# pytorch/audio

Hardware: AMD Instinct MI355X
Metric: audio-sec/sec MelSpectrogram (b=256, 16kHz, n_fft=400, n_mels=80) (higher is better)
Workload: dtype f32; 1 GPU; MelSpectrogram n_fft=400 hop=160 n_mels=80, batch=256 x 10 s @16 kHz fp32 per GPU (BASELINE configs[1]); per_gpu_batch=256

## Files before the change

### audio_amd/csrc/melspec400.h

```cpp
#pragma once
#include <cstdint>
#include <cstring>
#include <type_traits>
#include "hd.h"
#include "stft_generic.h"

namespace aamd {
namespace m400 {

constexpr int kN = 400;
constexpr int kPad = 200;
constexpr int kFramesPerWave = 6;
constexpr int kWavesPerBlock = 12;
constexpr int kMinWavesPerSimd = 3;
constexpr int kTOff[20] = {0, 260, 520, 652, 784, 916, 1444, 1576, 128, 388,
                           2104, 2232, 2364, 1708, 1840, 1048, 1180, 1312, 1972, 2492};
constexpr int kTBufDwords = 2492 + 128;
constexpr int kTRow = 44;
constexpr int kTPair = 20 * kTRow;
constexpr int kLdsDwordsPerWave = 3 * kTPair;
constexpr int kPK = 208;
constexpr int kPPair = 416;
constexpr int kSOff = 1344;

template <int H>
struct Hop {
  static constexpr int hop = 20 * H;
  static constexpr int nx = 20 + H;
  static constexpr int tile_samples = (kFramesPerWave - 1) * hop + kN;
  static constexpr int pair_stride = 2 * hop;
  static constexpr int pad = ((20 - pair_stride % 32) + 32) % 32;
  static constexpr int blk_data = pair_stride / 4, blk_pieces = blk_data + pad / 4;
  static constexpr int data_pieces = tile_samples / 4;
  static constexpr int pieces = data_pieces + (pad / 4) * ((tile_samples - 1) / pair_stride);
  static constexpr int ndma = (pieces + 63) / 64;
  static constexpr int lds_dwords = (kSOff + 256 * ndma > kLdsDwordsPerWave) ? kSOff + 256 * ndma : kLdsDwordsPerWave;
  static_assert(pad % 4 == 0 && (pair_stride + pad) % 32 == 20, "staging pad");
};
struct PcmStereo { uint32_t lr; };
template <typename TIn> struct InTraits {
  static constexpr int chans = 1;
  AAMD_HD static float get(const TIn* p, int) { return (float)*p; }
};
template <> struct InTraits<PcmStereo> {
  static constexpr int chans = 2;
  AAMD_HD static float get(const PcmStereo* p, int ch) { return (float)(int16_t)(uint16_t)(p->lr >> (16 * ch)); }
};

template <int H, typename TIn>
struct Stage {
  using HC = Hop<H>;
  static constexpr int spp = 16 / (int)sizeof(TIn);
  static constexpr int pair_dwords = HC::pair_stride * (int)sizeof(TIn) / 4;
  static constexpr int pad = sizeof(TIn) == 4 ? HC::pad : ((44 - pair_dwords % 64) + 64) % 64;
  static constexpr int pad_elems = pad * 4 / (int)sizeof(TIn);
  static constexpr int blk_data = HC::pair_stride / spp, blk_pieces = blk_data + pad / 4;
  static constexpr int data_pieces = HC::tile_samples / spp;
  static constexpr int pieces = data_pieces + (pad / 4) * ((HC::tile_samples - 1) / HC::pair_stride);
  static constexpr int ndma = (pieces + 63) / 64;
  static constexpr bool ok = (HC::pair_stride % spp == 0) && (HC::tile_samples % spp == 0) && (pad % 4 == 0) &&
                             (kSOff + 256 * ndma <= HC::lds_dwords);
};
static_assert(Stage<8, float>::blk_data == Hop<8>::blk_data && Stage<8, float>::blk_pieces == Hop<8>::blk_pieces &&
              Stage<8, float>::pieces == Hop<8>::pieces && Stage<8, float>::ndma == Hop<8>::ndma, "float staging = Hop");
static_assert(Stage<8, int16_t>::ok && Stage<8, int16_t>::pad == 12 && Stage<8, int16_t>::ndma == 3, "int16 staging, hop 160");
static_assert(Stage<10, int16_t>::ok && Stage<5, float>::ok && Stage<10, float>::ok, "staging geometry");
static_assert(sizeof(PcmStereo) == 4 && Stage<8, PcmStereo>::ok && Stage<10, PcmStereo>::ok &&
              Stage<8, PcmStereo>::pieces == Stage<8, float>::pieces, "interleaved stereo stages like float");

constexpr int kMelSlots = 20;
constexpr int kMelMaxRounds = 8;
constexpr int kMelMaxTaps = 64;

static_assert(3 * kPPair <= kLdsDwordsPerWave && 2 * kPK <= kPPair, "P rows must fit in the transposition buffer");
static_assert(kTBufDwords <= kLdsDwordsPerWave, "transposition rows must fit in the wave's region");
static_assert(3 * (kPK - 201) <= 64, "one lane per tail bin");
static_assert(Hop<8>::lds_dwords == kLdsDwordsPerWave && Hop<8>::ndma == 5 && Hop<8>::pad == 20, "headline geometry");

enum { EPI400_MEL = 0, EPI400_MEL_DB = 1, EPI400_SPEC = 2, EPI400_MEL_NORM = 3, EPI400_MFCC = 4 };
struct Epi400 {
  float multiplier, amin, db_sub;
  float* group_max;
  int64_t rows_per_group;
  float power;
  float gain;
  const float* mean;
  const float* invstd;
  int64_t out_frames;
  const float* dct_frag;
  int n_mfcc;
  float top_db;
  float* tile_min;
  int* fix_count;
  int* fix_list;
  int frag_in_lds;
  int fixup;
  int lab;
  unsigned* pool;
  int pool_p;
};
constexpr int kSpecBins = 201;

#ifndef AAMD_M400_POOLS
#define AAMD_M400_POOLS 0
#endif
constexpr int kPoolStride = 64;
constexpr unsigned kNoTile = 0xffffffffu;
AAMD_HD int pool_count(int nb) { return nb >= 8 ? nb / 8 : 1; }
AAMD_HD int pool_members(int nb, int np, int p) { return p < nb ? (nb - p + np - 1) / np : 0; }
AAMD_HD int pool_share(int tiles_per_block) { const int p = tiles_per_block / 20; return tiles_per_block < 48 ? 0 : p > 8 ? 8 : p; }
AAMD_HD unsigned pool_tile(int np, int P, int tiles_per_block, unsigned n_tiles, int p, int members, unsigned ticket,
                           bool& exhausted) {
  exhausted = ticket >= (unsigned)(members * P);
  if (exhausted) return kNoTile;
  const unsigned m = ticket / (unsigned)P, off = ticket - m * (unsigned)P;
  const unsigned long long t = (unsigned long long)(m * (unsigned)np + (unsigned)p) * (unsigned)tiles_per_block +
                               (unsigned)(tiles_per_block - P) + off;
  return t < n_tiles ? (unsigned)t : kNoTile;
}
static_assert(kFramesPerWave * kSpecBins + 3 <= kSOff && 3 * 2 * kSpecBins + 3 <= kSOff, "SPEC rows must fit below the staging area");

AAMD_HD constexpr int col_of_pos(int pi) {
  return pi == 0 ? 0 : pi == 1 ? 10 : (pi & 1) ? 20 - (pi >> 1) : (pi >> 1);
}
AAMD_HD constexpr int pos_of_col(int c) {
  return c == 0 ? 0 : c == 10 ? 1 : c < 10 ? 2 * c : 2 * (20 - c) + 1;
}

constexpr int kMfccMT = 3, kMfccMels = 80, kMfccSteps = 3;
constexpr float kMfccYScale = 1.0f / 16.0f, kMfccDScale = 16.0f;
static_assert(kMfccYScale * kMfccDScale == 1.0f, "the accumulators leave the matrix pipe unscaled");
constexpr int kMfccFragFloats = kMfccMT * kMfccSteps * 2 * 64 * 4;
AAMD_HD int mfcc_frag_piece(int t, int s, int hl, int lane) { return ((t * kMfccSteps + s) * 2 + hl) * 64 + lane; }
AAMD_HD int mfcc_slot_mel(int s, int lane, int j) {
  if (s < 2) return 32 * s + 8 * (lane >> 4) + j;
  return j < 4 ? 64 + 4 * (lane >> 4) + j : -1;
}
AAMD_HD float mfcc_frag_value(const float* dct, int n_mels, int n_mfcc, int t, int s, int lane, int j) {
  const int mel = mfcc_slot_mel(s, lane, j), coef = 16 * t + (lane & 15);
  return (mel >= 0 && mel < n_mels && coef < n_mfcc) ? dct[mel * n_mfcc + coef] * kMfccDScale : 0.0f;
}
AAMD_HD int mfcc_b_col_frame(int lane) { const int j = lane & 7; return j < kFramesPerWave ? j : kFramesPerWave - 1; }
AAMD_HD int mfcc_b_col_plane(int lane) { return (lane >> 3) & 1; }
AAMD_HD int mfcc_b_index(int lane, int s) {
  return mfcc_b_col_plane(lane) * (kFramesPerWave * kMfccMels) + mfcc_b_col_frame(lane) * kMfccMels +
         (s < 2 ? 32 * s + 8 * (lane >> 4) : 64 + 4 * (lane >> 4));
}
constexpr int kMfccPlaneHalves = kFramesPerWave * kMfccMels;

struct MelTab {
  const float* w;
  const int* lo2;
  const int* rc;
  const int* row_mel;
  int n_mels, ws, n_rounds;
};

AAMD_HD int mel_rounds(int n_mels) { return (n_mels + kMelSlots - 1) / kMelSlots; }
AAMD_HD int mel_ws(int max_width) {
  const int w4 = (max_width + 1 + 3) & ~3;
  return ((w4 >> 2) & 1) ? w4 : w4 + 4;
}
AAMD_HD int mel_rows(int n_mels) { return mel_rounds(n_mels) * kMelSlots; }
AAMD_HD int mel_tab_dwords(int n_mels, int max_width) {
  return mel_rows(n_mels) * (mel_ws(max_width) + 2) + kMelMaxRounds;
}
AAMD_HD int row_to_mel(const MelBandsDev& mb, int row) {
  const int m = mb.order ? mb.order[row] : row;
  return (m >= 0 && m < mb.n_mels) ? m : -1;
}

AAMD_HD void mel_tab_layout(const MelBandsDev& mb, float* base, MelTab& mt) {
  mt.n_mels = mb.n_mels;
  mt.ws = mel_ws(mb.max_width);
  mt.n_rounds = mel_rounds(mb.n_mels);
  const int rows = mel_rows(mb.n_mels);
  mt.w = base;
  int* lo2 = reinterpret_cast<int*>(base + rows * mt.ws);
  mt.lo2 = lo2;
  mt.row_mel = lo2 + rows;
  mt.rc = lo2 + 2 * rows;
}

AAMD_HD void mel_tab_rounds(int tid, int nthr, const MelBandsDev& mb, float* base, MelTab& mt) {
  mt.n_mels = mb.n_mels;
  mt.ws = mel_ws(mb.max_width);
  mt.n_rounds = mel_rounds(mb.n_mels);
  const int rows = mel_rows(mb.n_mels);
  mt.w = base;
  int* lo2 = reinterpret_cast<int*>(base + rows * mt.ws);
  int* row_mel = lo2 + rows;
  int* rc = row_mel + rows;
  mt.lo2 = lo2;
  mt.row_mel = row_mel;
  mt.rc = rc;
  for (int r = tid; r < mt.n_rounds; r += nthr) {
    int rw = 4;
    for (int row = r * kMelSlots; row < (r + 1) * kMelSlots; ++row) {
      const int q = row_to_mel(mb, row);
      if (q < 0) continue;
      const int e = (mb.width[q] + (mb.lo[q] & 1) + 3) & ~3;
      rw = e > rw ? e : rw;
    }
    rc[r] = rw >> 2;
  }
}

AAMD_HD void mel_tab_fill(int tid, int nthr, const MelBandsDev& mb, float* base, const MelTab& mt) {
  float* w = base;
  const int rows = mel_rows(mb.n_mels);
  int* lo2 = reinterpret_cast<int*>(base + rows * mt.ws);
  int* row_mel = lo2 + rows;
  for (int i = tid; i < rows * mt.ws; i += nthr) {
    const int row = i / mt.ws, j = i - row * mt.ws;
    const int m = row_to_mel(mb, row);
    const int rw = 4 * mt.rc[row / kMelSlots];
    const int lo = m >= 0 ? mb.lo[m] : 0, wd = m >= 0 ? mb.width[m] : 0;
    int l2 = lo & ~1;
    if (l2 + rw > kPK) l2 = kPK - rw;
    const int off = lo - l2;
    w[i] = (j >= off && j - off < wd) ? mb.weights[m * mb.max_width + (j - off)] : 0.0f;
    if (j == 0) {
      lo2[row] = l2;
      row_mel[row] = m;
    }
  }
}

constexpr int kTwRow = 42;
constexpr int kConstDwords = 20 * kTwRow + 20 * 20;

AAMD_HD void const_tab_build(int tid, int nthr, const float* window, const float* tw400, float scale,
                             float* base) {
  for (int i = tid; i < 20 * 20; i += nthr) {
    const int b = i / 20, s = i - 20 * b;
    const int idx = (b * s) % kN;
    base[kTwRow * b + 2 * s] = tw400[2 * idx];
    base[kTwRow * b + 2 * s + 1] = tw400[2 * idx + 1];
    base[20 * kTwRow + i] = window[b + 20 * s] * (0.5f * scale);
  }
}

AAMD_HD size_t lds_bytes(int n_mels, int max_width, int wave_dwords = kLdsDwordsPerWave, bool mfcc = false) {
  return ((size_t)kWavesPerBlock * wave_dwords + kConstDwords + mel_tab_dwords(n_mels, max_width) + 4 +
          (mfcc ? kMfccFragFloats : 0)) * sizeof(float);
}

struct LaneConst {
  const float* tw;
  const float* win;
  int p, pi, col;
  int active;
  int troff;
};

AAMD_HD void lane_init(int lane, const float* const_tab, LaneConst& c) {
  c.active = lane < 60;
  const int l = c.active ? lane : lane - 20;
  c.p = l / 20;
  c.pi = l - 20 * c.p;
  c.col = col_of_pos(c.pi);
  c.tw = const_tab + kTwRow * c.pi;
  c.win = const_tab + 20 * kTwRow + 20 * c.pi;
  int toff = 0;
#pragma unroll
  for (int k = 0; k < 20; ++k) toff = (c.col == k) ? kTOff[k] : toff;
  c.troff = toff + 20 * c.p;
}

AAMD_HD void dft4(float ar, float ai, float br, float bi, float cr, float ci, float dr, float di,
                  float* o_r, float* o_i) {
// ... 818 lines not shown
    for (int i = threadIdx.x; i < kMfccFragFloats; i += blockDim.x) frag_lds[i] = epi.dct_frag[i];
  if (EPI != EPI400_SPEC && mb.table400 != nullptr) {
    float* dst = const_tab + kConstDwords;
    for (int i = threadIdx.x; i < tab_dwords; i += blockDim.x) dst[i] = mb.table400[i];
    mel_tab_layout(mb, dst, mt);
    __syncthreads();
  } else {
    if (EPI != EPI400_SPEC) mel_tab_rounds(threadIdx.x, blockDim.x, mb, const_tab + kConstDwords, mt);
    __syncthreads();
    if (EPI != EPI400_SPEC) mel_tab_fill(threadIdx.x, blockDim.x, mb, const_tab + kConstDwords, mt);
    __syncthreads();
  }

  long long lab_t1 = 0;
  if (LAB & 1024) lab_t1 = wall_clock64();
  LaneConst c;
  lane_init(lane, const_tab, c);
  constexpr bool kWinRegs = (EPI != EPI400_MFCC || H != 10) && (((LAB & 8192) != 0) || !(LAB & 262144));
  float winr[20], twr[40];
  if (kWinRegs) {
#pragma unroll
    for (int q = 0; q < 20; ++q) winr[q] = c.win[q];
  }
  constexpr int kTwReg = 3, kTwRegPin = 4, kTwRegDb = 1, kTwRegMfcc = 2;
  constexpr bool kPlain = H == 8 && std::is_same<TIn, float>::value && LAB == 0;
  constexpr int kTwRegBatches = (LAB & 16384) ? 4
                                : (SIG != 0 && EPI == EPI400_MEL) ? ((AR & AR_PIN) ? kTwRegPin : kTwReg)
                                : !kPlain ? 0
                                : EPI == EPI400_SPEC ? 2
                                : (EPI == EPI400_MEL && SIG == 0) ? (NR <= 4 ? 1 : 3)
                                : (EPI == EPI400_MFCC && NR <= 4) ? kTwRegMfcc
                                : (EPI == EPI400_MEL_DB && NR <= 4) ? kTwRegDb : 0;
  if (kTwRegBatches > 0) {
#pragma unroll
    for (int q = 0; q < 10 * kTwRegBatches; ++q) twr[q] = c.tw[q];
  }
  constexpr bool kHoist = NR <= 4;
  MelRegs<NR> mregs;
  const MelRegs<NR>* mh = nullptr;
  if (EPI != EPI400_SPEC && kHoist) {
    mel_regs_load<NR>(c, mt, mregs);
    mh = &mregs;
  }
  if (SIG != 0) {
    static_assert(SIG == 0 || NR == 4, "filterbank signatures are 4 rounds of 20 mels");
    const int sig_rt = mregs.nc[0] | (mregs.nc[1 % NR] << 4) | (mregs.nc[2 % NR] << 8) | (mregs.nc[3 % NR] << 12);
    if (mt.n_rounds != NR || mt.n_mels != kMelSlots * NR || sig_rt != SIG) __builtin_trap();
  }
  if (EPI == EPI400_MFCC && (mt.n_rounds != NR || mt.n_mels != kMelSlots * NR)) __builtin_trap();
  float nrm_mean[NR], nrm_inv[NR];
  if (EPI == EPI400_MEL_NORM) {
#pragma unroll
    for (int r = 0; r < NR; ++r) {
      const int m = r < mt.n_rounds ? mt.row_mel[r * kMelSlots + c.pi] : -1;
      nrm_mean[r] = m >= 0 ? epi.mean[m] : 0.0f;
      nrm_inv[r] = m >= 0 ? epi.invstd[m] : 0.0f;
    }
  }
  const unsigned long long self_mask = __ballot((c.col == 0) || (c.col == 10));
  using SG = Stage<H, TIn>;
  static_assert(SG::ok, "no staging layout for this hop / input type");
  int spiece[SG::ndma];
#pragma unroll
  for (int k = 0; k < SG::ndma; ++k) spiece[k] = SG::spp * stage_src_piece<H, TIn>(64 * k + lane);

  const int nb = gridDim.x;
  int lb = blockIdx.x;
  if ((nb & 7) == 0) lb = (blockIdx.x & 7) * (nb >> 3) + (blockIdx.x >> 3);
  unsigned blk_first = (unsigned)lb * (unsigned)tiles_per_block;
  unsigned blk_count = 0;
  if (blk_first < (unsigned)n_tiles) {
    blk_count = (unsigned)n_tiles - blk_first;
    if (blk_count > (unsigned)tiles_per_block) blk_count = (unsigned)tiles_per_block;
  }
  if (EPI == EPI400_MFCC && epi.fixup != 0) {
    blk_first = 0;
    blk_count = fix_cnt;
  }
  const unsigned queue_addr = (unsigned)(uintptr_t)queue;
  auto claim = [&]() {
    int v = 0;
    if (lane == 0)
      asm volatile("ds_add_rtn_u32 %0, %1, %2\n\ts_waitcnt lgkmcnt(0)" : "=v"(v) : "v"(queue_addr), "v"(1) : "memory");
    return (unsigned)__builtin_amdgcn_readfirstlane(v);
  };
#if AAMD_M400_POOLS
#define AAMD_M400_POOLED (AAMD_M400_POOLS && (LAB == 0) && epi.pool != nullptr && !(EPI == EPI400_MFCC && epi.fixup != 0))
  if (AAMD_M400_POOLED && blk_count > (unsigned)(tiles_per_block - epi.pool_p)) blk_count = (unsigned)(tiles_per_block - epi.pool_p);
  unsigned pool_ticket = 0;
  auto pool_request = [&]() {
    int lbo = (int)(blk_first / (unsigned)tiles_per_block);
    asm volatile("" : "+s"(lbo));
    unsigned* const ctr = epi.pool + (lbo % pool_count(nb)) * kPoolStride;
    if (lane == 0) pool_ticket = __hip_atomic_fetch_add(ctr, 1u, __ATOMIC_RELAXED, __HIP_MEMORY_SCOPE_AGENT);
  };
  auto pool_take = [&]() {
    int lbo = (int)(blk_first / (unsigned)tiles_per_block);
    asm volatile("" : "+s"(lbo));
    const int np = pool_count(nb), pid = lbo % np, mem = pool_members(nb, np, pid);
    for (;;) {
      const unsigned v = (unsigned)__builtin_amdgcn_readfirstlane((int)pool_ticket);
      if (v + 1u == (unsigned)(mem * (epi.pool_p + kWavesPerBlock)) && lane == 0)
        __hip_atomic_store(epi.pool + pid * kPoolStride, 0u, __ATOMIC_RELAXED, __HIP_MEMORY_SCOPE_AGENT);
      bool exhausted;
      const unsigned t = pool_tile(np, epi.pool_p, tiles_per_block, (unsigned)n_tiles, pid, mem, v, exhausted);
      if (t != kNoTile) return t - blk_first;
      if (exhausted) return 0x80000000u;
      pool_request();
    }
  };
  constexpr unsigned kBadIdx = 0x80000000u, kPendIdx = 0x80000001u;
#define AAMD_M400_IDX_OK(I) ((((I) ^ 0x80000000u)) > 1u)
#define AAMD_M400_LOCAL(I) ((I) < blk_count ? (I) : kBadIdx)
#else
#define AAMD_M400_IDX_OK(I) ((I) < blk_count)
#define AAMD_M400_LOCAL(I) (I)
#endif
  constexpr unsigned kLabChunk = 8;
  unsigned* gq = reinterpret_cast<unsigned*>(epi.group_max);
  int g_pending = 0;
  unsigned g_base = 0, g_pos = 0;
  auto g_request = [&]() {
    if (lane == 0) g_pending = (int)__hip_atomic_fetch_add(gq, 1u, __ATOMIC_RELAXED, __HIP_MEMORY_SCOPE_AGENT);
  };
  if (LAB & 131072) {
    blk_count = (unsigned)n_tiles;
    g_request();
    g_base = (unsigned)__builtin_amdgcn_readfirstlane(g_pending) * kLabChunk;
    g_request();
  }
  auto g_next = [&]() {
    if (++g_pos < kLabChunk) return g_base + g_pos;
    g_base = (unsigned)__builtin_amdgcn_readfirstlane(g_pending) * kLabChunk;
    g_pos = 0;
    g_request();
    return g_base;
  };

  static_assert(kFramesPerWave * kHop >= kPad, "tile 1 starts inside the clip");
  unsigned tin_hi = 0;
  if (in_aligned && length >= kN - kPad) {
    int64_t last = (length - (kN - kPad)) / kHop - (kFramesPerWave - 1);
    if (last > (int64_t)n_frames - kFramesPerWave) last = (int64_t)n_frames - kFramesPerWave;
    if (last >= kFramesPerWave) tin_hi = (unsigned)(last / kFramesPerWave);
  }
  const int64_t out_row_elems =
      EPI == EPI400_SPEC   ? (int64_t)n_frames * (epi.power > 0.0f ? kSpecBins : 2 * kSpecBins)
      : EPI == EPI400_MFCC ? (int64_t)n_frames * epi.n_mfcc
                           : (EPI == EPI400_MEL_NORM ? epi.out_frames : (int64_t)n_frames) * (int64_t)mb.n_mels;
  auto tile_fill = [&](TileInfo& ti, unsigned idx) {
    ti.t0 = (int)ti.tin * kFramesPerWave;
    ti.staged = AAMD_M400_IDX_OK(idx) && ti.tin - 1u < tin_hi;
  };
  auto tile_info = [&](unsigned idx) {
    TileInfo ti;
    unsigned t = ((LAB & 131072) ? 0u : blk_first) + idx;
    if (EPI == EPI400_MFCC && epi.fixup != 0)
      t = idx < blk_count ? (unsigned)__hip_atomic_load(epi.fix_list + fix_base + idx, __ATOMIC_RELAXED, __HIP_MEMORY_SCOPE_AGENT) : 0u;
    const unsigned row = t / (unsigned)tiles_per_row;
    ti.row = row;
    ti.tin = t - row * (unsigned)tiles_per_row;
    ti.in_off = (ti.row / InTraits<TIn>::chans) * row_stride;
    ti.out_off = ti.row * out_row_elems;
    tile_fill(ti, idx);
    return ti;
  };
  constexpr bool kCarry = !(LAB & (131072 | 16777216)) && !AAMD_M400_POOLS && EPI != EPI400_MFCC && InTraits<TIn>::chans == 1;
  constexpr unsigned kCarryMinTiles = 16;
  auto tile_next = [&](const TileInfo& from, unsigned from_idx, unsigned idx) {
    if (!kCarry || (unsigned)tiles_per_row < kCarryMinTiles) return tile_info(idx);
    TileInfo ti = from;
    if (!(AAMD_M400_IDX_OK(idx))) {
      ti.staged = false;
      return ti;
    }
    ti.tin = from.tin + (idx - from_idx);
    while (ti.tin >= (unsigned)tiles_per_row) {
      ti.tin -= (unsigned)tiles_per_row;
      ti.row += 1;
      ti.in_off += row_stride;
      ti.out_off += out_row_elems;
    }
    tile_fill(ti, idx);
    return ti;
  };
  auto stage_issue = [&](const TileInfo& ti) {
    const TIn* src = wav + ti.in_off + ((int64_t)ti.t0 * kHop - kPad);
    if (LAB & 32) src = wav + 6 * kHop;
#pragma unroll
    for (int k = 0; k < SG::ndma; ++k)
      if (!(LAB & 64) || k == 0)
        glds16s(src, (unsigned)spiece[k] * (unsigned)sizeof(TIn), s_addr + 1024 * k);
  };

  float wmax = -INFINITY;
  int64_t wgroup = -1, wrow = -1;
  constexpr bool kDb = (EPI == EPI400_MEL_DB) || (EPI == EPI400_MFCC);
  const bool fix = (EPI == EPI400_MFCC) && epi.fixup != 0;
  auto flush_max = [&]() {
    if (kDb && !fix && epi.group_max != nullptr && wgroup >= 0) {
      float m = wmax;
#pragma unroll
      for (int off = 32; off > 0; off >>= 1) m = fmaxf(m, __shfl_xor(m, off, 64));
      if (lane == 0) atomic_max_f32(epi.group_max + wgroup, m);
    }
    wmax = -INFINITY;
  };

  if (kIoWave && wave >= kWavesPerBlock - kNio) {
    constexpr unsigned D = 8;
    constexpr bool kFetchOnly = (LAB & 134217728) != 0;
    if (!(LAB & 33554432)) {
      const unsigned n_mine = (blk_count + (unsigned)kNio - 1u - (unsigned)(wave - (kWavesPerBlock - kNio))) / (unsigned)kNio;
      for (unsigned i = 0; i < n_mine + D; ++i) {
        const unsigned t = i * (unsigned)kNio + (unsigned)(wave - (kWavesPerBlock - kNio));
        if (i < n_mine) {
          const TileInfo ti = tile_info(AAMD_M400_LOCAL(t));
          const unsigned dst = (unsigned)(uintptr_t)(smem400 + (t % (unsigned)kWavesPerBlock) * HC::lds_dwords + kSOff);
          if (ti.staged) {
            const TIn* src = wav + ti.in_off + ((int64_t)ti.t0 * kHop - kPad);
#pragma unroll
            for (int k = 0; k < SG::ndma; ++k) glds16(src + spiece[k], dst + 1024 * k);
          }
        }
        if (i >= D) {
          if (kFetchOnly) {
            asm volatile("s_waitcnt vmcnt(40)" ::: "memory");
          } else {
            asm volatile("s_waitcnt vmcnt(56)" ::: "memory");
            const unsigned told = t - D * (unsigned)kNio;
            const TileInfo to = tile_info(AAMD_M400_LOCAL(told));
            const float* stg = smem400 + (told % (unsigned)kWavesPerBlock) * HC::lds_dwords;
            store_wide(lane, mt, stg, out + to.row * (int64_t)n_frames * (int64_t)mb.n_mels, to.t0, n_frames);
          }
        }
      }
    }
    blk_count = 0;
  }
  unsigned cur_idx = (LAB & 131072) ? g_base : (unsigned)wave;
#if AAMD_M400_POOLS
  if (cur_idx >= blk_count) cur_idx = kBadIdx;
  if (AAMD_M400_POOLED && cur_idx == kBadIdx) {
    pool_request();
    cur_idx = pool_take();
  }
#endif
  TileInfo cur = tile_info(cur_idx);
  if (LAB & 128) {
    const int k = (wave + 6 * lb) % 3;
    for (int i = 0; i < k; ++i) __builtin_amdgcn_s_sleep(112);
  }
  if (LAB & 2048) {
    const int k = 4 * (wave & 3) + (wave >> 2) % 3;
    for (int i = 0; i < (k % 12); ++i) __builtin_amdgcn_s_sleep(17);
  }
  if (LAB & 4096) {
    const int k = 4 * ((wave >> 2) % 3) + (wave & 3);
    for (int i = 0; i < k; ++i) __builtin_amdgcn_s_sleep(17);
  }
  float Xn[HC::nx];
  auto gload = [&](const TileInfo& ti) {
    const TIn* src = wav + ti.in_off + ((int64_t)ti.t0 * kHop - kPad) + (HC::pair_stride * c.p + c.pi);
#pragma unroll
    for (int q = 0; q < HC::nx; ++q) Xn[q] = InTraits<TIn>::get(src + 20 * q, (int)(ti.row % InTraits<TIn>::chans));
  };
  if (LAB & 32768) {
#pragma unroll
    for (int q = 0; q < HC::nx; ++q) Xn[q] = 0.0f;
    if (cur.staged) gload(cur);
  } else if (cur.staged && !(LAB & 8) && !fix) {
    stage_issue(cur);
  }

  long long ph_acc[6] = {0, 0, 0, 0, 0, 0}, ph_t = 0;
  int ph_tiles = 0;
#define AAMD_M400_STAMP(K)                                  \
  if (LAB & 8388608) {                                      \
    const long long now_ = (long long)clock64();            \
    ph_acc[K] += now_ - ph_t;                               \
    ph_t = now_;                                            \
  }
  using mfcc_f32x4 = __attribute__((ext_vector_type(4))) float;
  mfcc_f32x4 cf[kMfccMT];
  const int mfcc_elab = (LAB & 524288) ? epi.lab : 0;
  auto mfcc_finish = [&](int64_t row, int64_t t0) {
#pragma unroll
    for (int t = 0; t < kMfccMT; ++t)
#pragma unroll
      for (int i = 0; i < 4; ++i) {
        cf[t][i] += __int_as_float(__builtin_amdgcn_mov_dpp(__float_as_int(cf[t][i]), 0x128, 0xf, 0xf, true));
        asm volatile("" : "+v"(cf[t][i]));
      }
    const int64_t left64 = n_frames - t0;
    const int left = left64 < kFramesPerWave ? (int)left64 : kFramesPerWave;
    if (!(LAB & 2) && !(mfcc_elab & 8) && (lane & 15) < left) {
      float* otile = out + (row * (int64_t)n_frames + t0) * (int64_t)epi.n_mfcc;
      const unsigned ooff = (unsigned)(lane & 15) * (unsigned)epi.n_mfcc + 4u * (unsigned)(lane >> 4);
#pragma unroll
      for (int t = 0; t < kMfccMT; ++t) {
        const int k0 = 16 * t + 4 * (lane >> 4);
        if (k0 < epi.n_mfcc) *reinterpret_cast<F4*>(otile + (ooff + 16u * (unsigned)t)) = F4{cf[t][0], cf[t][1], cf[t][2], cf[t][3]};
      }
    }
  };
  while (AAMD_M400_IDX_OK(cur_idx)) {
    if (LAB & 8388608) { ph_t = (long long)clock64(); ++ph_tiles; }
#if AAMD_M400_POOLS
    unsigned nxt_idx = (LAB & 131072) ? g_next() : claim();
    if (nxt_idx >= blk_count) nxt_idx = AAMD_M400_POOLED ? kPendIdx : kBadIdx;
#else
    const unsigned nxt_idx = (LAB & 131072) ? g_next() : claim();
#endif
    TileInfo nxt = tile_next(cur, cur_idx, nxt_idx);
    float fix_cut = -INFINITY;
    if (fix) {
      fix_cut = epi.group_max[cur.row / epi.rows_per_group] - epi.top_db;
      if (cur.staged) stage_issue(cur);
    }

    float X[HC::nx];
    if ((LAB & 32768) && cur.staged) {
#pragma unroll
      for (int q = 0; q < HC::nx; ++q) X[q] = Xn[q];
    } else if (cur.staged) {
      if (!(LAB & 1)) stage_wait();
      if (LAB & 256) {
#pragma unroll
        for (int q = 0; q < HC::nx; ++q) X[q] = (float)(q + lane) * scale;
      } else {
        gather_lds<H, TIn>(c, reinterpret_cast<const TIn*>(lds + kSOff), X, (int)(cur.row % InTraits<TIn>::chans));
      }
    } else {
      gather_global<H, TIn>(c, wav + cur.in_off, length, cur.t0, n_frames, X,
                            (int)(cur.row % InTraits<TIn>::chans));
    }
#if AAMD_M400_POOLS
    if (nxt_idx == kPendIdx) pool_request();
#endif
    phase_a<H, kWinRegs, kTwRegBatches, AR>(c, X, lds, winr, twr);
    if ((LAB & 32768) && nxt.staged) gload(nxt);
    wave_lds_fence();
    AAMD_M400_STAMP(0)
    float vr[20], vi[20], zr[20], zi[20], qr[10], qi[10];
    phase_b1_load(c, lds, vr, vi);
    if (!(LAB & 32768)) {
      asm volatile("s_waitcnt lgkmcnt(0)" ::: "memory");
      AAMD_M400_STAMP(1)
#if AAMD_M400_POOLS
      if (nxt_idx == kPendIdx) {
        nxt_idx = pool_take();
        nxt = tile_info(nxt_idx);
      }
#endif
      if (nxt.staged && !(LAB & 8) && !fix) stage_issue(nxt);
    }
    if (LAB & 16) { wave_lds_fence(); cur = nxt; cur_idx = nxt_idx; continue; }
    dft20<(AR & AR_PIN) != 0, kDft2U1iMask>(vr, vi, zr, zi);
    phase_b2_send(c, zr, zi, qr, qi);
    exchange_partner(qr, qi, self_mask);
    wave_lds_fence();
    AAMD_M400_STAMP(2)
    if (EPI == EPI400_SPEC) {
      const int64_t left = n_frames - cur.t0;
      const int n_valid = left < kFramesPerWave ? (int)left : kFramesPerWave;
      if (epi.power > 0.0f) {
        const int64_t a0 = cur.out_off + (int64_t)cur.t0 * kSpecBins;
        phase_b2_spec(c, zr, zi, qr, qi, epi.power, (int)(a0 & 3), lds);
        wave_lds_fence();
        if (!(LAB & 2)) {
          if (n_valid == kFramesPerWave) store_spec_full(lane, lds, out, a0);
          else store_spec(lane, lds, out, a0, n_valid * kSpecBins);
        }
        wave_lds_fence();
      } else {
#pragma unroll
        for (int half = 0; half < 2; ++half) {
          const int64_t a0 = cur.out_off + (int64_t)(cur.t0 + 3 * half) * (2 * kSpecBins);
          const int nv = n_valid - 3 * half < 3 ? n_valid - 3 * half : 3;
          phase_b2_spec_complex(c, zr, zi, qr, qi, half, (int)(a0 & 3), lds);
          wave_lds_fence();
          if (!(LAB & 2) && nv > 0) store_spec(lane, lds, out, a0, nv * 2 * kSpecBins);
          wave_lds_fence();
        }
      }
      cur = nxt;
      cur_idx = nxt_idx;
      continue;
    }
    phase_b2<AR>(c, zr, zi, qr, qi, lds);
    phase_b2_pad(lane, lds);
    wave_lds_fence();
    AAMD_M400_STAMP(3)
    float acc_a[NR], acc_b[NR];
    if (LAB & 4) { wave_lds_fence(); cur = nxt; cur_idx = nxt_idx; continue; }
    phase_c<NR, SIG, EPI == EPI400_MFCC, (AR & AR_PK_BAND) != 0>(c, mt, lds, acc_a, acc_b, mh);
    if (LAB & 8388608) { asm volatile("" : "+v"(acc_a[0]), "+v"(acc_b[NR - 1])); }
    AAMD_M400_STAMP(4)
    if (kDb) {
      if (cur.row != wrow) {
        wrow = cur.row;
        const int64_t g = cur.row / epi.rows_per_group;
        if (g != wgroup) {
          flush_max();
          wgroup = g;
        }
      }
      const bool va_ok = cur.t0 + 2 * c.p < n_frames, vb_ok = cur.t0 + 2 * c.p + 1 < n_frames;
      float tmin = INFINITY;
      if (EPI == EPI400_MFCC) {
        const float db_c1 = epi.multiplier * 0.30102999566398120f;
#pragma unroll
        for (int r = 0; r < NR; ++r) {
          acc_a[r] = __builtin_fmaf(__log2f(vmax_raw(acc_a[r], epi.amin)), db_c1, -epi.db_sub);
          acc_b[r] = __builtin_fmaf(__log2f(vmax_raw(acc_b[r], epi.amin)), db_c1, -epi.db_sub);
        }
        if (cur.t0 + kFramesPerWave <= n_frames) {
#pragma unroll
          for (int r = 0; r < NR; ++r) {
            wmax = vmax3_raw(wmax, acc_a[r], acc_b[r]);
            tmin = vmin3_raw(tmin, acc_a[r], acc_b[r]);
          }
        } else {
#pragma unroll
          for (int r = 0; r < NR; ++r) {
            wmax = fmaxf(wmax, fmaxf(va_ok ? acc_a[r] : -INFINITY, vb_ok ? acc_b[r] : -INFINITY));
            tmin = fminf(tmin, fminf(va_ok ? acc_a[r] : INFINITY, vb_ok ? acc_b[r] : INFINITY));
          }
        }
        if (fix) {
#pragma unroll
          for (int r = 0; r < NR; ++r) {
            acc_a[r] = vmax_raw(acc_a[r], fix_cut);
            acc_b[r] = vmax_raw(acc_b[r], fix_cut);
          }
        }
      } else {
        const bool interior = cur.t0 + kFramesPerWave <= n_frames;
#pragma unroll
        for (int r = 0; r < NR; ++r) {
          if (r < mt.n_rounds) {
            acc_a[r] = epi.multiplier * fast_log10(vmax_raw(acc_a[r], epi.amin)) - epi.db_sub;
            acc_b[r] = epi.multiplier * fast_log10(vmax_raw(acc_b[r], epi.amin)) - epi.db_sub;
            if (interior) wmax = vmax3_raw(wmax, acc_a[r], acc_b[r]);
            else wmax = fmaxf(wmax, fmaxf(va_ok ? acc_a[r] : -INFINITY, vb_ok ? acc_b[r] : -INFINITY));
          }
        }
      }
      if (EPI == EPI400_MFCC && !fix && !(elab & 4)) {
        asm volatile(
            "s_nop 1\n\t"
            "v_min_f32_dpp %0, %0, %0 row_shr:1 row_mask:0xf bank_mask:0xf\n\ts_nop 1\n\t"
            "v_min_f32_dpp %0, %0, %0 row_shr:2 row_mask:0xf bank_mask:0xf\n\ts_nop 1\n\t"
            "v_min_f32_dpp %0, %0, %0 row_shr:4 row_mask:0xf bank_mask:0xf\n\ts_nop 1\n\t"
            "v_min_f32_dpp %0, %0, %0 row_shr:8 row_mask:0xf bank_mask:0xf\n\ts_nop 1\n\t"
            "v_min_f32_dpp %0, %0, %0 row_bcast:15 row_mask:0xa bank_mask:0xf\n\ts_nop 1\n\t"
            "v_min_f32_dpp %0, %0, %0 row_bcast:31 row_mask:0xc bank_mask:0xf"
            : "+v"(tmin));
        if (lane == 63) epi.tile_min[blk_first + cur_idx] = tmin;
      }
    }
    if (EPI == EPI400_MFCC) {
      using f32x4 = __attribute__((ext_vector_type(4))) float;
      using h8 = __attribute__((ext_vector_type(8))) _Float16;
      using h4 = __attribute__((ext_vector_type(4))) _Float16;
      using u32x4 = __attribute__((ext_vector_type(4))) uint32_t;
      using u32x2 = __attribute__((ext_vector_type(2))) uint32_t;
      wave_lds_fence();
      {
        uint16_t* hs = reinterpret_cast<uint16_t*>(lds);
        uint16_t* ls = hs + kMfccPlaneHalves;
#pragma unroll
        for (int r = 0; r < NR; ++r) {
          const int m = mh ? mh->mel(r) : mt.row_mel[r * kMelSlots + c.pi];
          const float va = acc_a[r] * kMfccYScale, vb = acc_b[r] * kMfccYScale;
          const _Float16 ha = (_Float16)va, hb = (_Float16)vb;
          const _Float16 la = (_Float16)(va - (float)ha), lb = (_Float16)(vb - (float)hb);
          hs[2 * c.p * kMfccMels + m] = __builtin_bit_cast(uint16_t, ha);
          ls[2 * c.p * kMfccMels + m] = __builtin_bit_cast(uint16_t, la);
          hs[(2 * c.p + 1) * kMfccMels + m] = __builtin_bit_cast(uint16_t, hb);
          ls[(2 * c.p + 1) * kMfccMels + m] = __builtin_bit_cast(uint16_t, lb);
        }
      }
      wave_lds_fence();
#pragma unroll
      for (int t = 0; t < kMfccMT; ++t) cf[t] = f32x4{0.0f, 0.0f, 0.0f, 0.0f};
      auto product = [&](const u32x4* __restrict__ ftab) {
        const uint16_t* hs = reinterpret_cast<const uint16_t*>(lds);
        u32x4 a0[kMfccMT][2];
        auto frag_load = [&](int sidx) {
#pragma unroll
          for (int t = 0; t < kMfccMT; ++t)
#pragma unroll
            for (int hl = 0; hl < 2; ++hl) {
              a0[t][hl] = u32x4{0x3c003c00u, 0x3c003c00u, 0x3c003c00u, 0x3c003c00u};
              if (!(elab & 1)) a0[t][hl] = ftab[mfcc_frag_piece(t, sidx, hl, lane)];
            }
        };
#pragma unroll
        for (int sidx = 0; sidx < 2; ++sidx) {
          const h8 bb = __builtin_bit_cast(h8, *reinterpret_cast<const u32x4*>(hs + mfcc_b_index(lane, sidx)));
          frag_load(sidx);
#pragma unroll
          for (int t = 0; t < kMfccMT; ++t)
            cf[t] = __builtin_amdgcn_mfma_f32_16x16x32_f16(__builtin_bit_cast(h8, a0[t][1]), bb, cf[t], 0, 0, 0);
#pragma unroll
          for (int t = 0; t < kMfccMT; ++t)
            cf[t] = __builtin_amdgcn_mfma_f32_16x16x32_f16(__builtin_bit_cast(h8, a0[t][0]), bb, cf[t], 0, 0, 0);
        }
        {
          frag_load(2);
          const h4 bb = __builtin_bit_cast(h4, *reinterpret_cast<const u32x2*>(hs + mfcc_b_index(lane, 2)));
#define AAMD_A4(T, HL) __builtin_bit_cast(h4, u32x2{a0[T][HL][0], a0[T][HL][1]})
#pragma unroll
          for (int t = 0; t < kMfccMT; ++t) cf[t] = __builtin_amdgcn_mfma_f32_16x16x16f16(AAMD_A4(t, 1), bb, cf[t], 0, 0, 0);
#pragma unroll
          for (int t = 0; t < kMfccMT; ++t) cf[t] = __builtin_amdgcn_mfma_f32_16x16x16f16(AAMD_A4(t, 0), bb, cf[t], 0, 0, 0);
#undef AAMD_A4
        }
      };
      if (!(elab & 2)) {
        if (kFragLds) product(reinterpret_cast<const u32x4*>(frag_lds));
        else product(reinterpret_cast<const u32x4*>(epi.dct_frag));
      }
      if (!(elab & 2)) mfcc_finish(cur.row, cur.t0);
      wave_lds_fence();
      cur = nxt;
      cur_idx = nxt_idx;
      continue;
    }
    if (EPI == EPI400_MEL_NORM) {
#pragma unroll
      for (int r = 0; r < NR; ++r) {
        if (r < mt.n_rounds) {
          acc_a[r] = (epi_plog(acc_a[r] * epi.gain) - nrm_mean[r]) * nrm_inv[r];
          acc_b[r] = (epi_plog(acc_b[r] * epi.gain) - nrm_mean[r]) * nrm_inv[r];
        }
      }
    }
    float* out_row = out + cur.out_off;
    if (LAB & 4194304) out_row = out + (int64_t)(wave + kWavesPerBlock * (blockIdx.x & 63)) * 6 * mb.n_mels - cur.t0 * (int64_t)mb.n_mels;
    if (out_wide) {
      wave_lds_fence();
      store_stage<NR>(c, mt, acc_a, acc_b, lds, mh);
      wave_lds_fence();
      if (!(LAB & 2)) store_wide(lane, mt, lds, out_row, cur.t0, n_frames);
    } else {
      if (!(LAB & 2)) store_direct<NR, SIG>(c, mt, acc_a, acc_b, out_row, cur.t0, n_frames, mh);
    }
    wave_lds_fence();
    AAMD_M400_STAMP(5)
    cur = nxt;
    cur_idx = nxt_idx;
  }
#undef AAMD_M400_STAMP
  if ((LAB & 8388608) && lane == 0) {
    long long* rec = reinterpret_cast<long long*>(epi.fix_count) + 4 * 12 * 256 + 8 * (blockIdx.x * kWavesPerBlock + wave);
#pragma unroll
    for (int k = 0; k < 6; ++k) rec[k] = ph_acc[k];
    rec[6] = ph_tiles;
  }
  if (kDb && !fix && epi.group_max != nullptr) {
    float m = wmax;
#pragma unroll
    for (int off = 32; off > 0; off >>= 1) m = fmaxf(m, __shfl_xor(m, off, 64));
    if (lane == 0) {
      reinterpret_cast<int*>(lds)[0] = (int)wgroup;
      lds[1] = m;
    }
    __syncthreads();
    if (threadIdx.x == 0) {
      int g_run = -1;
      float m_run = -INFINITY;
      for (int w = 0; w < kWavesPerBlock; ++w) {
        const int gw = reinterpret_cast<const int*>(smem400 + w * HC::lds_dwords)[0];
        const float mw = smem400[w * HC::lds_dwords + 1];
        if (gw != g_run) {
          if (g_run >= 0) atomic_max_f32(epi.group_max + g_run, m_run);
          g_run = gw;
          m_run = mw;
        } else {
          m_run = fmaxf(m_run, mw);
        }
      }
      if (g_run >= 0) atomic_max_f32(epi.group_max + g_run, m_run);
    }
  }
  if ((LAB & 1048576) && lane == 0) {
    long long* rec = reinterpret_cast<long long*>(epi.fix_count);
    const int w = blockIdx.x * kWavesPerBlock + wave;
    rec[4 * w + 2] = (long long)clock64();
    rec[4 * w + 3] = wall_clock64();
  }
  if ((LAB & 1024) && lane == 0) {
    long long* rec = reinterpret_cast<long long*>(const_cast<float*>(tw400) + 1024);
    const int w = blockIdx.x * kWavesPerBlock + wave;
    rec[3 * w] = lab_t0;
    rec[3 * w + 1] = lab_t1;
    rec[3 * w + 2] = wall_clock64();
  }
}
#endif

}
}
```

Measured before the change: 37.01 million audio-sec/sec.

## Process unstaged edge tiles first within each block's tile range

Reorders the tiles each block processes so the unstaged edge tiles (first and last tiles of each row, which go through the slower global gather) are claimed before the staged interior tiles. Index mapping helpers compute the row and tile-in-row for the reordered sequence, and the carry logic wraps over interior tiles only. The aim is to keep slow tiles out of the tail of the schedule so wave completion is more even. The change also adds extra index arithmetic, a fresh tile_info call after each unstaged gather, keys tile_min writes by absolute tile position, and adds some debug recording under a lab flag.

Result: slower. 36.26 million audio-sec/sec (-2.0%).

```diff
diff --git a/audio_amd/csrc/melspec400.h b/audio_amd/csrc/melspec400.h
--- a/audio_amd/csrc/melspec400.h
+++ b/audio_amd/csrc/melspec400.h
@@ -117,6 +117,40 @@
   const unsigned long long t = (unsigned long long)(m * (unsigned)np + (unsigned)p) * (unsigned)tiles_per_block +
                                (unsigned)(tiles_per_block - P) + off;
   return t < n_tiles ? (unsigned)t : kNoTile;
+}
+
+struct RunTile { unsigned row, tin; };
+AAMD_HD unsigned run_staged_before(unsigned t, unsigned tpr, unsigned tin_hi) {
+  const unsigned row = t / tpr, tin = t - row * tpr;
+  const unsigned in_row = tin == 0 ? 0u : (tin - 1u < tin_hi ? tin - 1u : tin_hi);
+  return row * tin_hi + in_row;
+}
+AAMD_HD unsigned run_unstaged(unsigned first, unsigned count, unsigned tpr, unsigned tin_hi) {
+  return count - (run_staged_before(first + count, tpr, tin_hi) - run_staged_before(first, tpr, tin_hi));
+}
+AAMD_HD bool run_edge_first(unsigned n_unstaged, unsigned tin_hi) { return tin_hi != 0 && n_unstaged <= (unsigned)kWavesPerBlock; }
+AAMD_HD RunTile run_tile(unsigned idx, unsigned first, unsigned n_unstaged, unsigned staged_first, unsigned tpr,
+                         unsigned tin_hi) {
+  RunTile r;
+  if (idx < n_unstaged) {
+    const unsigned per_row = tpr - tin_hi, k = (first - staged_first) + idx;
+    r.row = k / per_row;
+    const unsigned j = k - r.row * per_row;
+    r.tin = j == 0 ? 0u : tin_hi + j;
+  } else {
+    const unsigned k = staged_first + (idx - n_unstaged);
+    r.row = k / tin_hi;
+    r.tin = 1u + (k - r.row * tin_hi);
+  }
+  return r;
+}
+AAMD_HD RunTile run_carry(unsigned row, unsigned tin, unsigned dist, unsigned hi, unsigned period) {
+  RunTile r{row, tin + dist};
+  while (r.tin > hi) {
+    r.tin -= period;
+    r.row += 1;
+  }
+  return r;
 }
 static_assert(kFramesPerWave * kSpecBins + 3 <= kSOff && 3 * 2 * kSpecBins + 3 <= kSOff, "SPEC rows must fit below the staging area");
 
@@ -1241,14 +1275,28 @@
     ti.t0 = (int)ti.tin * kFramesPerWave;
     ti.staged = AAMD_M400_IDX_OK(idx) && ti.tin - 1u < tin_hi;
   };
+  constexpr bool kEdgeFirst = !AAMD_M400_POOLS && !(LAB & (131072 | 16777216 | 268435456));
+  bool edge_first = false;
+  unsigned ord_unstaged = 0, ord_staged_first = 0;
+  if (kEdgeFirst && tin_hi != 0 && !(EPI == EPI400_MFCC && epi.fixup != 0)) {
+    ord_unstaged = run_unstaged(blk_first, blk_count, (unsigned)tiles_per_row, tin_hi);
+    edge_first = run_edge_first(ord_unstaged, tin_hi);
+    ord_staged_first = run_staged_before(blk_first, (unsigned)tiles_per_row, tin_hi);
+  }
   auto tile_info = [&](unsigned idx) {
     TileInfo ti;
-    unsigned t = ((LAB & 131072) ? 0u : blk_first) + idx;
-    if (EPI == EPI400_MFCC && epi.fixup != 0)
-      t = idx < blk_count ? (unsigned)__hip_atomic_load(epi.fix_list + fix_base + idx, __ATOMIC_RELAXED, __HIP_MEMORY_SCOPE_AGENT) : 0u;
-    const unsigned row = t / (unsigned)tiles_per_row;
-    ti.row = row;
-    ti.tin = t - row * (unsigned)tiles_per_row;
+    if (edge_first) {
+      const RunTile rt = run_tile(idx, blk_first, ord_unstaged, ord_staged_first, (unsigned)tiles_per_row, tin_hi);
+      ti.row = rt.row;
+      ti.tin = rt.tin;
+    } else {
+      unsigned t = ((LAB & 131072) ? 0u : blk_first) + idx;
+      if (EPI == EPI400_MFCC && epi.fixup != 0)
+        t = idx < blk_count ? (unsigned)__hip_atomic_load(epi.fix_list + fix_base + idx, __ATOMIC_RELAXED, __HIP_MEMORY_SCOPE_AGENT) : 0u;
+      const unsigned row = t / (unsigned)tiles_per_row;
+      ti.row = row;
+      ti.tin = t - row * (unsigned)tiles_per_row;
+    }
     ti.in_off = (ti.row / InTraits<TIn>::chans) * row_stride;
     ti.out_off = ti.row * out_row_elems;
     tile_fill(ti, idx);
@@ -1256,6 +1304,7 @@
   };
   constexpr bool kCarry = !(LAB & (131072 | 16777216)) && !AAMD_M400_POOLS && EPI != EPI400_MFCC && InTraits<TIn>::chans == 1;
   constexpr unsigned kCarryMinTiles = 16;
+  const unsigned carry_end = edge_first ? tin_hi + 1u : (unsigned)tiles_per_row;
   auto tile_next = [&](const TileInfo& from, unsigned from_idx, unsigned idx) {
     if (!kCarry || (unsigned)tiles_per_row < kCarryMinTiles) return tile_info(idx);
     TileInfo ti = from;
@@ -1264,8 +1313,8 @@
       return ti;
     }
     ti.tin = from.tin + (idx - from_idx);
-    while (ti.tin >= (unsigned)tiles_per_row) {
-      ti.tin -= (unsigned)tiles_per_row;
+    while (ti.tin >= carry_end) {
+      ti.tin -= edge_first ? tin_hi : (unsigned)tiles_per_row;
       ti.row += 1;
       ti.in_off += row_stride;
       ti.out_off += out_row_elems;
@@ -1393,8 +1442,11 @@
       }
     }
   };
+  unsigned lab_last_idx = 0, lab_tiles = 0;
+  bool lab_last_unstaged = false;
   while (AAMD_M400_IDX_OK(cur_idx)) {
     if (LAB & 8388608) { ph_t = (long long)clock64(); ++ph_tiles; }
+    if (LAB & 1048576) { lab_last_idx = cur_idx; lab_last_unstaged = !cur.staged; ++lab_tiles; }
 #if AAMD_M400_POOLS
     unsigned nxt_idx = (LAB & 131072) ? g_next() : claim();
     if (nxt_idx >= blk_count) nxt_idx = AAMD_M400_POOLED ? kPendIdx : kBadIdx;
@@ -1423,6 +1475,7 @@
     } else {
       gather_global<H, TIn>(c, wav + cur.in_off, length, cur.t0, n_frames, X,
                             (int)(cur.row % InTraits<TIn>::chans));
+      if (kCarry && edge_first && (unsigned)tiles_per_row >= kCarryMinTiles) nxt = tile_info(nxt_idx);
     }
 #if AAMD_M400_POOLS
     if (nxt_idx == kPendIdx) pool_request();
@@ -1546,7 +1599,7 @@
             "v_min_f32_dpp %0, %0, %0 row_bcast:15 row_mask:0xa bank_mask:0xf\n\ts_nop 1\n\t"
             "v_min_f32_dpp %0, %0, %0 row_bcast:31 row_mask:0xc bank_mask:0xf"
             : "+v"(tmin));
-        if (lane == 63) epi.tile_min[blk_first + cur_idx] = tmin;
+        if (lane == 63) epi.tile_min[(unsigned)cur.row * (unsigned)tiles_per_row + cur.tin] = tmin;
       }
     }
     if (EPI == EPI400_MFCC) {
@@ -1680,6 +1733,13 @@
     const int w = blockIdx.x * kWavesPerBlock + wave;
     rec[4 * w + 2] = (long long)clock64();
     rec[4 * w + 3] = wall_clock64();
+    if (!(LAB & 8388608)) {
+      long long* last = rec + 4 * 12 * 256 + 8 * w;
+      last[0] = lab_last_idx;
+      last[1] = lab_tiles;
+      last[2] = lab_last_unstaged ? 1 : 0;
+      last[3] = blk_count;
+    }
   }
   if ((LAB & 1024) && lane == 0) {
     long long* rec = reinterpret_cast<long long*>(const_cast<float*>(tw400) + 1024);
```
